# lab-cosmo/torch-pme

Hardware: AMD Instinct MI355X
Metric: atom-steps/sec (energy+forces) (higher is better)
Workload: dtype f32

## Files before the change

### torch-pme_amd/csrc/bricks.hip

```cpp
#include "bricks_device.h"

namespace mipme {
bool bricks_supported(const mipme_mesh_t* m, int dtype) {
  const size_t s = dtype == MIPME_F32 ? 4 : 8;
  const int ns[3] = {m->nx, m->ny, m->nz};
  for (int d = 0; d < 3; ++d) {
    if (ns[d] <= 2 * BRICK) return false;
    const int rem = ns[d] % BRICK;
    if (rem != 0 && rem < 4) return false;
  }
  const size_t tile = BRICK + m->order - 1;
  if (2 * size_t(m->n_channels) * tile * tile * tile * s > 60 * 1024) return false;
  if (spread_stage_rows(m->order, s) == 0) return false;
  return true;
}
int64_t bins_bytes(const mipme_mesh_t* m, int64_t N, int dtype) {
  if (!bricks_supported(m, dtype)) return 0;
  return int64_t(bins_layout(m, N, dtype).total);
}
int plane_bins_capacity(const mipme_mesh_t* m, int64_t N, int dtype) { return plane_list_capacity(m, N, dtype); }
int plane_bands(const mipme_mesh_t* m, int dtype) {
  const int rows = plane_band_rows(m, dtype);
  return rows > 0 ? m->ny / rows : 0;
}
const void* bins_epart(const mipme_mesh_t* m, int64_t N, int dtype, void* bins, int64_t* n) {
  *n = (N + 64 / kRowLanes - 1) / (64 / kRowLanes);
  return bins_view(m, N, dtype, bins).epart;
}

bool plane_spread_runs(const mipme_mesh_t* m, int64_t N, int dtype, const mipme_sr_job_t* job, const PlaneHost* ph, bool forward) {
  const int pcap = plane_list_capacity(m, N, dtype);
  const int band_rows = pcap > 0 ? plane_band_rows(m, dtype) : 0;
  const bool bands_ok = band_rows == m->ny || !job || (job->shift_format & kShiftFormatMask) == kShiftTable32;
  return ph && ph->hat && ph->slot_values && !ph->keep_mesh && forward && pcap > 0 && m->n_channels == 1 &&
         !sparse_bricks(N, make_brick_geom(m).nb) && !deterministic_mode() && N > 0 && band_rows > 0 && bands_ok;
}

static bool defer_slots_setting() {
  static const bool on = env_flag("MIPME_DEFER_SLOTS", true);
  return on;
}
bool bins_defer_slots(const mipme_mesh_t* m, int64_t N, int dtype, const mipme_sr_job_t* job, const PlaneHost* ph) {
  return defer_slots_setting() && N < kCoalescedBinAtoms && plane_spread_runs(m, N, dtype, job, ph, true);
}
SlotRider bins_slot_rider(const mipme_mesh_t* m, int64_t N, int dtype, void* bins, const void* pos, const void* q) {
  const BinsView v = bins_view(m, N, dtype, bins);
  SlotRider r;
  r.n_atoms = N;
  r.scheme = m->scheme;
  r.order = m->order;
  r.g = make_geom(m);
  r.pos = pos;
  r.q = q;
  r.dst = v.dst;
  r.rec = v.rec;
  r.wts = v.wts;
  r.qs = v.qs;
  r.codes = v.idx.codes;
  r.over_base = v.idx.over_base;
  return r;
}

template <typename T>
int bins_build(hipStream_t st, const mipme_mesh_t* m, int64_t n_atoms, const void* pos, void* bins, int* live,
               const void* q, void* atom_rec, bool plane_lists, bool defer_slots) {
  const int dtype = dtype_of<T>();
  const Geom g = make_geom(m);
  const BrickGeom bg = make_brick_geom(m);
  BinsView v = bins_view(m, n_atoms, dtype, bins);
  MIPME_REQUIRE(live, "the binning pass needs the live brick counters");
  if (plane_lists && v.idx.pcap > 0 && !deterministic_mode()) {
// ... 364 lines not shown
```

### torch-pme_amd/csrc/common.h

```cpp
#pragma once

#include <hip/hip_runtime.h>
#include <cstdarg>
#include <cstdint>
#include <cstdlib>
#include <cstdio>

#include "../../include/mipme.h"

namespace mipme {

void set_error(const char* fmt, ...);
void note_cosched_kernel(const char* name);
void note_slot_fill(int rider_atoms);
void note_cell_riders(int n);

#define MIPME_CHECK_HIP(expr)                                                                 \
  do {                                                                                        \
    hipError_t _e = (expr);                                                                   \
    if (_e != hipSuccess) {                                                                   \
      mipme::set_error("%s failed: %s (%s:%d)", #expr, hipGetErrorString(_e), __FILE__, __LINE__); \
      return MIPME_EHIP;                                                                      \
    }                                                                                         \
  } while (0)
// ... 259 lines not shown
    for (int off = 32; off > 0; off >>= 1) tot += __shfl_xor(tot, off, 64);
    if (threadIdx.x == 0) work[k] = tot;
  }
  if (threadIdx.x == 0) __hip_atomic_store(counter, 0, __ATOMIC_RELAXED, __HIP_MEMORY_SCOPE_AGENT);
}

struct SlotRider {
  int64_t n_atoms = 0;
  int per_rider = 0;
  int scheme = 0, order = 0;
  Geom g;
  const void* pos = nullptr;
  const void* q = nullptr;
  const int* dst = nullptr;
  int4* rec = nullptr;
  void* wts = nullptr;
  void* qs = nullptr;
  unsigned char* codes = nullptr;
  int64_t over_base = 0;
};

struct ConvCell {
  const void* G_deriv;
  const double* cwave;
  int64_t n_waves;
  void* wbuf;
  double* rows;
  int n_riders;
  void* rho_hat_out;
  const void* rho_hat_in;
  double* kh_rows;
  int* ticket;
  const SlotRider* slots = nullptr;
};

struct PlaneHost {
  void* hat = nullptr;
  bool keep_mesh = true;
  bool slot_values = false;
  int parts = 1;
  void* hat_more = nullptr;
  int64_t more_stride = 0;
  mutable int parts_used = 1;
  mutable bool ycols_pending = false;
};
struct RowRideHost {
  const mipme_sr_job_t* job;
  void* epart;
  int64_t first_row, n_rows;
};

__host__ __device__ __forceinline__ unsigned xcd_contiguous(unsigned wg, unsigned n_items) {
  const unsigned chunk = (n_items + 7u) >> 3;
  return (wg & 7u) * chunk + (wg >> 3);
}
__host__ __device__ __forceinline__ unsigned pad8(unsigned n) { return (n + 7u) & ~7u; }

inline const int*& skip_flag_slot() {
  static thread_local const int* p = nullptr;
  return p;
}
#define MIPME_SKIP_IF_SET(ptr)                          \
  do {                                                  \
    if ((ptr) != nullptr && *(ptr) == 1) return;        \
  } while (0)

// ... 42 lines not shown
```

### torch-pme_amd/csrc/frames.hip

```cpp
#include "frames_device.h"

namespace mipme {
template <int SCHEME, int N, typename T>
__global__ __launch_bounds__(256) void frames_bin_atoms_kernel(const FrameDev<T>* __restrict__ table) {
  const FrameDev<T>& f = table[blockIdx.y];
  if (int64_t(blockIdx.x) * 256 >= f.N) return;
  bin_atoms_body<SCHEME, N, T>(f.g, f.bg, f.bins, f.N, f.pos, f.over_brick, f.rec, f.wts, f.q, f.atom_rec, blockIdx.x, nullptr,
                               const_cast<T*>(f.spread.qs));
}

template <int N, typename T, int PFAST, bool COMPACT>
__global__ __launch_bounds__(SPREAD_THREADS, (sizeof(T) == 4 && COMPACT) ? 6 : 1) void frames_spread_rows_kernel(const FrameDev<T>* __restrict__ table) {
  const FrameDev<T>& f = table[blockIdx.y];
  const unsigned n_spread = unsigned(f.bg.nb);
  if (blockIdx.x < n_spread)
    spread_brick_body<N, T>(f.spread, blockIdx.x);
  else if (blockIdx.x - n_spread < f.n_row_blocks) {
    extern __shared__ __attribute__((aligned(16))) char smem_rows[];
    AtomRecord<T>* tab = reinterpret_cast<AtomRecord<T>*>(smem_rows);
    if constexpr (COMPACT && std::is_same<T, float>::value) {
      if (!f.rows.dist_out) {
        sr_rows_pk_body<PFAST, SPREAD_THREADS>(f.rows, blockIdx.x - n_spread, tab);
        return;
      }
// ... 107 lines not shown
                  "frame %d: the frames path needs the table shift format (1 or 2), the same for every frame", k);
  }
  return MIPME_OK;
}

template <typename T>
static int frames_table_build_t(int n_frames, const mipme_frame_t* fr, const mipme_potential_t* pot, void* host_table) {
  SRPot s;
  int rc = make_srpot(pot, s);
  if (rc) return rc;
  const int pfast = fast_rs_exponent(s);
  MIPME_REQUIRE(pot->smearing > 0 && (pfast == 1 || pfast == 6), "the frames path covers 1/r and 1/r^6 with a smearing");
  const FastRS cf = make_fast_rs(s);
  double self_c, bg_c;
  correction_terms(pot, self_c, bg_c);
  const int dtype = dtype_of<T>();
  FrameDev<T>* out = (FrameDev<T>*)host_table;
  for (int k = 0; k < n_frames; ++k) {
    const mipme_frame_t& f = fr[k];
    const mipme_mesh_t* m = &f.mesh;
    const BinsView v = bins_view(m, f.n_atoms, dtype, f.atom_bins);
    FrameDev<T> d;
    d.g = make_geom(m);
    d.bg = make_brick_geom(m);
    d.N = f.n_atoms;
    d.pos = (const T*)f.positions;
    d.q = (const T*)f.charges;
    d.bins = v.idx;
    d.bins.live = (int*)f.brick_counters;
    d.over_brick = v.over_brick;
    d.rec = v.rec;
    d.wts = (T*)v.wts;
    d.atom_rec = (AtomRecord<T>*)f.records;
    d.even = (m->order % 2) == 0;
    d.spread.g = d.g;
    d.spread.bg = d.bg;
    d.spread.C = 1;
    d.spread.bins = d.bins;
    d.spread.from_live = true;
    d.spread.rec = v.rec;
    d.spread.wts = (const T*)v.wts;
    d.spread.val = (const T*)f.charges;
    d.spread.scale = T(1);
    d.spread.mesh = (T*)f.rho_mesh;
    d.spread.stage_rows = spread_stage_rows(m->order, sizeof(T));
    d.spread.skip = nullptr;
    d.spread.det = false;
    d.spread.qs = (const T*)v.qs;
    if (frame_plane_lists(f, dtype)) {
      d.bins.plive = d.bins.live + d.bg.nb + 1;
    } else {
      d.bins.pcap = 0;
      d.bins.wmax = nullptr;
    }
    d.spread.bins = d.bins;
    d.rows = make_fused_rows_args<T>(s, cf, f.n_atoms, f.row_ptr, f.entries_shift, f.entries, nullptr, f.positions, f.records,
                                     f.cell, f.charges, nullptr, 0, f.full_list ? 0 : 1, f.full_list, 0, f.out, f.force, nullptr,
                                     f.dist_out);
    const int64_t rpb = SPREAD_THREADS / kRowLanes;
    d.n_row_blocks = unsigned((f.n_atoms + rpb - 1) / rpb);
    d.phi_mesh = (const T*)f.phi_mesh;
    d.dc = (const T*)f.dc;
    d.inv_vol = T(1.0 / m->volume);
    d.self_c = T(self_c);
    d.bg_c = T(bg_c);
    d.out = (T*)f.out;
// ... 7 lines not shown
    th.force_scale = f.full_list ? 0.5 : 1.0;
    th.seed = f.grad_seed;
    th.grad_pos = f.grad_positions;
    th.energy = f.energy;
    d.tail = make_gather_tail<T>(th, v.epart, int((f.n_atoms + 64 / kRowLanes - 1) / (64 / kRowLanes)), nullptr, nullptr);
    d.use_tail = f.use_tail != 0;
    d.rows.epart = f.use_tail ? v.epart : nullptr;
    out[k] = d;
  }
  return MIPME_OK;
}

template <typename T>
static FrameCellRec* frames_cell_recs(const void* table, int n_frames) {
  static_assert(sizeof(FrameDev<T>) % 8 == 0, "the cell records follow the frame records");
  return (FrameCellRec*)((char*)const_cast<void*>(table) + size_t(n_frames) * sizeof(FrameDev<T>));
}

template <typename T>
static int frames_forward_t(mipme_fft_plan* plan, hipStream_t st, int n_frames, const mipme_frame_t* fr, const void* table,
                            const void* G, int64_t G_stride, void* rho_all, void* hat_all, void* phi_all, void* dc_all,
                            int pfast, void* cell_work = nullptr, bool slab = false) {
  const FrameDev<T>* tb = (const FrameDev<T>*)table;
  const mipme_mesh_t* m = &fr[0].mesh;
  const BrickGeom bg = make_brick_geom(m);
  int64_t max_atoms = 0;
  for (int k = 0; k < n_frames; ++k) max_atoms = std::max<int64_t>(max_atoms, fr[k].n_atoms);
  const unsigned atom_blocks = unsigned((max_atoms + 255) / 256);
  const unsigned F = unsigned(n_frames);
  if (slab) {
    const int rcs = frames_slab_moments<T>(st, tb, n_frames, max_atoms);
    if (rcs) return rcs;
  }
  MIPME_DISPATCH_STENCIL_B(m->scheme, m->order, (frames_bin_atoms_kernel<S, N, T><<<dim3(atom_blocks, F), 256, 0, st>>>(tb)));
  MIPME_LAUNCH_CHECK();
  const int stage_rows = spread_stage_rows(m->order, sizeof(T));
  const size_t lds = spread_lds_bytes(m->order, sizeof(T), stage_rows);
  const int64_t rpb = SPREAD_THREADS / kRowLanes;
  const unsigned grid_x = unsigned(bg.nb) + unsigned((max_atoms + rpb - 1) / rpb);
  const bool compact = fr[0].shift_format == kShiftTable32;
  bool planes = fft_plan_plane_forward_ok_batched(plan);
  for (int k = 0; k < n_frames && planes; ++k) planes = frame_plane_lists(fr[k], dtype_of<T>());
  fft_plan_begin_step(plan);
  int rc0 = MIPME_OK;
  if (!planes) note_cosched_kernel("frames_spread_rows_kernel");
  if (planes) {
    PlaneArgs<T> pa;
    size_t need = 0;
    plane_lds_layout<T>(m->ny, m->nz, pa, need);
    const int64_t Mh = int64_t(m->nx) * m->ny * (m->nz / 2 + 1);
    pa.hat = (Cplx<T>*)hat_all;
    pa.parts = plane_spread_parts_setting();
    while (pa.parts > 1 && int64_t(pa.parts) * m->nx * n_frames > 128) --pa.parts;
    if (pa.parts > 1) {
      pa.hat_more = (Cplx<T>*)fft_plan_hat_parts(plan, st, kPlanePartsMax - 1);
      pa.more_stride = Mh * n_frames;
      if (!pa.hat_more) pa.parts = 1;
    }
    while ((1 << pa.logny) < m->ny) ++pa.logny;
    while ((1 << pa.loglz) < m->nz / 2) ++pa.loglz;
    const size_t rows_lds = sizeof(T) * size_t(SPREAD_WAVES) * BRICK_PTS;
    const size_t plds = need > rows_lds ? need : rows_lds;
    const unsigned pgrid_x = unsigned(m->nx) * unsigned(pa.parts) + unsigned((max_atoms + rpb - 1) / rpb);
#define MIPME_FRAMES_PLANES(PF, CO) \
  MIPME_DISPATCH_STENCIL_B(m->scheme, m->order, (frames_plane_rows_kernel<S, N, T, PF, CO><<<dim3(pgrid_x, F), SPREAD_THREADS, plds, st>>>(tb, pa, Mh)))
    note_cosched_kernel("frames_plane_rows_kernel");
    if (cell_work) {
      if ((rc0 = frames_cell_plane_rows<T>(st, m->scheme, m->order, pfast, dim3(pgrid_x, F), plds, tb, pa, Mh))) return rc0;
    } else if (pfast == 1 && compact)
      MIPME_FRAMES_PLANES(1, true);
    else if (pfast == 1)
      MIPME_FRAMES_PLANES(1, false);
    else if (compact)
      MIPME_FRAMES_PLANES(6, true);
    else
      MIPME_FRAMES_PLANES(6, false);
#undef MIPME_FRAMES_PLANES
    fft_plan_set_forward_done(plan, true, pa.parts);
  } else if (cell_work) {
    if ((rc0 = frames_cell_spread_rows<T>(st, m->scheme, m->order, pfast, dim3(grid_x, F), lds, tb))) return rc0;
  } else if (pfast == 1 && compact)
    MIPME_DISPATCH_STENCIL_B(m->scheme, m->order,
                             ((void)S, frames_spread_rows_kernel<N, T, 1, true><<<dim3(grid_x, F), SPREAD_THREADS, lds, st>>>(tb)));
  else if (pfast == 1)
    MIPME_DISPATCH_STENCIL_B(m->scheme, m->order,
                             ((void)S, frames_spread_rows_kernel<N, T, 1, false><<<dim3(grid_x, F), SPREAD_THREADS, lds, st>>>(tb)));
  else if (compact)
    MIPME_DISPATCH_STENCIL_B(m->scheme, m->order,
                             ((void)S, frames_spread_rows_kernel<N, T, 6, true><<<dim3(grid_x, F), SPREAD_THREADS, lds, st>>>(tb)));
  else
    MIPME_DISPATCH_STENCIL_B(m->scheme, m->order,
                             ((void)S, frames_spread_rows_kernel<N, T, 6, false><<<dim3(grid_x, F), SPREAD_THREADS, lds, st>>>(tb)));
  MIPME_LAUNCH_CHECK();
  bool all_tail = true;
  for (int k = 0; k < n_frames; ++k) all_tail = all_tail && fr[k].use_tail != 0;
  const int64_t n_k = xconv_blocks(plan) / n_frames;
  void* epart_k = nullptr;
  int rc;
  if (all_tail && (rc = fft_plan_tail_scratch(plan, int64_t(sizeof(double)) * n_k * n_frames, &epart_k))) return rc;
  ConvCell cc{};
  cc.wbuf = cell_work;
  rc = convolve_xfused(plan, st, rho_all, G, hat_all, phi_all, dc_all, G_stride, nullptr, nullptr, nullptr, epart_k, nullptr, 0, nullptr, nullptr,
                       cell_work ? &cc : nullptr);
  if (rc) return rc;
  const FrameCellRec* recs = frames_cell_recs<T>(table, n_frames);
  if (cell_work) {
    MIPME_REQUIRE(all_tail, "the cell gradient of a frame batch rides on the gather tail of every frame");
    const int n_riders = int(cell_work_layout(m, 1, nullptr).n_riders);
    if ((rc = frames_cell_riders<T>(st, recs, n_frames, n_riders, m->nx, m->ny, m->nz / 2 + 1, (const double*)epart_k, int(n_k)))) return rc;
  }
  if (slab) {
    MIPME_REQUIRE(all_tail, "the slab term of a frame batch rides on the gather tail of every frame");
    if ((rc = frames_slab_gather_tail<T>(st, m->scheme, m->order, dim3(unsigned(bg.nb), F), tb, (const double*)epart_k, int(n_k)))) return rc;
    return cell_work ? frames_slab_cell_finalize<T>(st, recs, n_frames) : MIPME_OK;
  }
  if (all_tail) {
    MIPME_DISPATCH_STENCIL_B(m->scheme, m->order,
                             ((void)S, frames_gather_tail_kernel<N, T><<<dim3(unsigned(bg.nb), F), GATHER_THREADS, 0, st>>>(
                                 tb, (const double*)epart_k, int(n_k))));
    MIPME_LAUNCH_CHECK();
    if (cell_work) return frames_cell_finalize<T>(st, recs, n_frames);
    return MIPME_OK;
  }
  MIPME_DISPATCH_STENCIL_B(m->scheme, m->order,
                           ((void)S, frames_gather_kernel<N, T><<<dim3(unsigned(bg.nb), F), GATHER_THREADS, 0, st>>>(tb)));
  MIPME_LAUNCH_CHECK();
  frames_energy_kernel<T><<<F, 1024, 0, st>>>(tb);
  MIPME_LAUNCH_CHECK();
  return MIPME_OK;
}

}

using namespace mipme;

template <typename T>
static int frames_table_energy_log_t(int n_frames, void* host_table, void* log, void* cursors, int capacity) {
// ... 269 lines not shown
```

### torch-pme_amd/csrc/frames_device.h

```cpp
#pragma once
#include "bricks_device.h"

namespace mipme {
template <typename T>
struct FrameDev {
  Geom g;
  BrickGeom bg;
  int64_t N;
  const T* pos;
  const T* q;
  BinIndex bins;
  int* over_brick;
  int4* rec;
  T* wts;
  AtomRecord<T>* atom_rec;
  int even;
  SpreadArgs<T> spread;
  FusedRowsArgs<T> rows;
  unsigned n_row_blocks;
  const T* phi_mesh;
  const T* dc;
  T inv_vol, self_c, bg_c;
  T* out;
  T* field;
  T* energy;
  const T* force;
  T* grad_pos;
  T force_scale;
  GatherTail<T> tail;
  bool use_tail;
};

template <typename T> int frames_cell_plane_rows(hipStream_t st, int scheme, int order, int pfast, dim3 grid, size_t lds,
                                                 const FrameDev<T>* table, const PlaneArgs<T>& pa, int64_t frame_stride);
template <typename T> int frames_cell_spread_rows(hipStream_t st, int scheme, int order, int pfast, dim3 grid, size_t lds, const FrameDev<T>* table);

template <typename T> int frames_slab_moments(hipStream_t st, const FrameDev<T>* table, int n_frames, int64_t max_atoms);
template <typename T> int frames_slab_gather_tail(hipStream_t st, int scheme, int order, dim3 grid, const FrameDev<T>* table,
                                                  const double* epart_k, int n_k);

}
```

### torch-pme_amd/csrc/host.h

```cpp
#pragma once

#include <algorithm>
#include <climits>
#include <cmath>
#include <cstring>

#include "common.h"

namespace mipme {

template <typename T>
constexpr int dtype_of() {
  return sizeof(T) == 4 ? MIPME_F32 : MIPME_F64;
}

#define DT_SWITCH(dtype, CALL_F32, CALL_F64)                    \
  do {                                                          \
    if ((dtype) == MIPME_F32) return CALL_F32;                  \
    if ((dtype) == MIPME_F64) return CALL_F64;                  \
    mipme::set_error("invalid dtype %d", int(dtype));           \
    return MIPME_EINVAL;                                        \
  } while (0)

inline unsigned stride_grid(int64_t n, int block) {
// ... 58 lines not shown
int64_t cellgrad_blocks(const mipme_mesh_t* m);
int64_t cellgrad_scratch_doubles();
template <typename T> int cellgrad_finalize_impl(hipStream_t st, const mipme_mesh_t* m, double bg, int64_t n_atoms, void* partials,
                                                 const void* pos, const void* grad_pos, const void* gout, const void* phi_atoms,
                                                 const void* rho_dc, const void* psi_dc, const void* energy_scale, void* grad_cell,
                                                 int64_t kgrid_blocks, const void* field, const void* q);
template <typename T> int cell_tail_finalize_impl(hipStream_t st, const mipme_mesh_t* m, double bg, double pair_scale, int64_t n_rows,
                                                  int64_t n_bricks, const void* rows, const void* rpart, const void* dc, const void* seed, void* out,
                                                  const GatherTailHost* slab = nullptr);

template <typename T, typename I> int rspace_forward_impl(hipStream_t st, int64_t P, int64_t N, int C, const void* pairs, const void* dist, const void* q,
                                                          const void* mask, int full, const mipme_potential_t* pot, int accumulate, void* out);
template <typename T, typename I> int rspace_backward_impl(hipStream_t st, int64_t P, int64_t N, int C, const void* pairs, const void* dist,
                                                           const void* q, const void* mask, int full, const mipme_potential_t* pot, const void* g,
                                                           const void* gscale, void* grad_d, void* grad_q);
template <typename T, typename I> int distance_forward_impl(hipStream_t st, int64_t P, const void* pairs, const void* pos, const void* cell,
                                                            const void* shifts, void* out);
template <typename T, typename I> int distance_backward_impl(hipStream_t st, int64_t P, int64_t N, const void* pairs, const void* pos, const void* cell,
                                                             const void* shifts, const void* grad_d, void* partials, void* grad_pos, void* grad_cell);
template <typename T> int pack_pair_shifts_impl(hipStream_t st, int64_t P, const void* shifts, void* packed, void* flag);
template <typename T> int distance_forward_packed_impl(hipStream_t st, int64_t P, const void* pairs, const void* packed, const void* pos,
                                                       const void* cell, void* out);
int64_t pair_partials_blocks(int64_t P);

bool bricks_supported(const mipme_mesh_t* m, int dtype);
int64_t bins_bytes(const mipme_mesh_t* m, int64_t N, int dtype);
int plane_bins_capacity(const mipme_mesh_t* m, int64_t N, int dtype);
int plane_bands(const mipme_mesh_t* m, int dtype);
const void* bins_epart(const mipme_mesh_t* m, int64_t N, int dtype, void* bins, int64_t* n);
bool sr_job_fusable(const mipme_sr_job_t* job);
template <typename T> int bins_build(hipStream_t st, const mipme_mesh_t* m, int64_t n_atoms, const void* pos, void* bins, int* live,
                                     const void* q, void* atom_rec, bool plane_lists = false, bool defer_slots = false);
bool plane_spread_runs(const mipme_mesh_t* m, int64_t N, int dtype, const mipme_sr_job_t* job, const PlaneHost* ph, bool forward);
bool bins_defer_slots(const mipme_mesh_t* m, int64_t N, int dtype, const mipme_sr_job_t* job, const PlaneHost* ph);
SlotRider bins_slot_rider(const mipme_mesh_t* m, int64_t N, int dtype, void* bins, const void* pos, const void* q);
template <typename T> int spread_bricks(hipStream_t st, const mipme_mesh_t* m, int64_t N, void* bins, const void* val, double scale, void* mesh,
                                        int* clear_count, const mipme_sr_job_t* job, bool want_epart, double* cpart, const PlaneHost* ph = nullptr,
                                        bool* used_planes = nullptr);
template <typename T> int gather_bricks(hipStream_t st, const mipme_mesh_t* m, int64_t N, void* bins, const void* mesh, const void* q,
                                        const void* qsum, double self_c, double bg_c, void* out, void* raw, int accumulate, void* field,
                                        const GatherTailHost* th, void* nan_flag, int* live);
template <typename T> int gather_grad_bricks(hipStream_t st, const mipme_mesh_t* m, int64_t N, void* bins, const void* q, const void* gout,
                                             const void* phi, const void* chi, const void* psi_dc, const void* gscale, double self_c,
                                             double bg_c, void* grad_pos, void* grad_q);

bool live_supported(const mipme_mesh_t* m, int64_t N, int dtype);
int64_t live_lists_ints(const mipme_mesh_t* m, int64_t N);
template <typename T> int live_rebin(hipStream_t st, const mipme_mesh_t* m, int64_t N, const void* rec4, void* bins, void* lists, void* host_flags);
template <typename T> int live_spread(hipStream_t st, const mipme_mesh_t* m, int64_t N, const void* rec4, void* bins, void* lists, void* mesh,
                                      const mipme_sr_job_t* job, void* host_flags, double* cpart);
template <typename T> int live_gather(hipStream_t st, const mipme_mesh_t* m, int64_t N, const void* rec4, void* bins, void* lists, const void* mesh,
                                      const void* qsum, double self_c, double bg_c, void* out, void* field, const GatherTailHost* th, void* nan_flag);

inline void correction_terms(const mipme_potential_t* pot, double& self_c, double& bg_c) {
  const int p = pot->kind == MIPME_COULOMB ? 1 : pot->exponent;
  const double two_s2 = 2.0 * pot->smearing * pot->smearing;
  self_c = pot->prefactor / std::tgamma(0.5 * p + 1.0) / std::pow(two_s2, 0.5 * p);
  if (p >= 3)
    bg_c = 0.0;
  else
    bg_c = pot->prefactor * std::pow(3.14159265358979323846, 1.5) * std::pow(two_s2, 0.5 * (3 - p)) /
           ((3 - p) * std::tgamma(0.5 * p));
}

static constexpr int kPlanePartsMax = 8;
inline int plane_spread_parts_setting() {
// ... 91 lines not shown
```

### torch-pme_amd/csrc/kfilter.hip

```cpp
#include <hipfft/hipfft.h>

#include <cmath>
#include <cstdlib>
#include <new>

#include "host.h"
#include "kgrid.h"
#include "kpot.h"
#include "fft_lds.h"
#include "cell_finalize_device.h"
#include "bricks_device.h"

namespace mipme {

struct KPoint {
  double k[3];
  int f[3];
  double G, dGdk[3], dGdh[3];
  double alpha, beta[3];
};

__device__ inline void eval_point(const KGeom& g, const KPot& kp, int ix, int iy, int iz, KPoint& o) {
  o.f[0] = fft_freq(ix, g.nx);
  o.f[1] = fft_freq(iy, g.ny);
  o.f[2] = iz;
  const double k2 = kvector_dev(g.inv, o.f, o.k);
  double v, dv;
  lr_kernel_dev(kp, k2, v, dv);
  if (g.scheme == MIPME_LAGRANGE) {
    o.G = v;
    o.alpha = 2.0 * dv;
#pragma unroll
    for (int c = 0; c < 3; ++c) {
      o.dGdk[c] = 2.0 * o.k[c] * dv;
      o.dGdh[c] = 0.0;
      o.beta[c] = 0.0;
    }
    return;
  }
  double s = 1.0, t[3], sn[3], cs[3];
#pragma unroll
  for (int c = 0; c < 3; ++c) {
    t[c] = 0.5 * o.k[c] * g.h[c];
    sincos(t[c], &sn[c], &cs[c]);
// ... 409 lines not shown

template <typename T, bool INVERSE, bool YSTAGE = true>
__global__ __launch_bounds__(1024) void yz_planes_kernel(int ny, int nz, int logny, int loglz, const T* __restrict__ real_in,
                                                       Cplx<T>* __restrict__ hat, T* __restrict__ real_out,
                                                       const int* __restrict__ skip, unsigned n_planes, CellRider rider) {
  MIPME_SKIP_IF_SET(skip);
  extern __shared__ __attribute__((aligned(16))) char smem_yz[];
  if constexpr (INVERSE && YSTAGE) {
    if (blockIdx.x >= n_planes) {
      cell_rider_body<T>(rider, blockIdx.x - n_planes, int(blockDim.x), reinterpret_cast<double*>(smem_yz));
      return;
    }
  }
  yz_plane_body<T, INVERSE, YSTAGE>(ny, nz, logny, loglz, real_in, hat, real_out, blockIdx.x, smem_yz);
}

template <int SCHEME, int N, typename T>
__global__ __launch_bounds__(1024) void yz_planes_slots_kernel(int ny, int nz, int logny, int loglz, Cplx<T>* __restrict__ hat,
                                                             T* __restrict__ real_out, const int* __restrict__ skip,
                                                             unsigned n_planes, CellRider rider, SlotRider slots) {
  MIPME_SKIP_IF_SET(skip);
  extern __shared__ __attribute__((aligned(16))) char smem_yz[];
  if (blockIdx.x >= n_planes + unsigned(rider.n_riders)) {
    slot_rider_body<SCHEME, N, T>(slots, blockIdx.x - n_planes - unsigned(rider.n_riders));
    return;
  }
  if (blockIdx.x >= n_planes) {
    cell_rider_body<T>(rider, blockIdx.x - n_planes, int(blockDim.x), reinterpret_cast<double*>(smem_yz));
    return;
  }
  yz_plane_body<T, true, true>(ny, nz, logny, loglz, nullptr, hat, real_out, blockIdx.x, smem_yz);
}

__device__ __forceinline__ unsigned xcd_tile(unsigned b, unsigned n) {
  const unsigned x = b & 7u, per = n >> 3, rem = n & 7u;
  return x * per + (x < rem ? x : rem) + (b >> 3);
}

template <typename T, bool INVERSE>
__global__ __launch_bounds__(256) void ycols_kernel(int ny, int nzh, int logny, int kzs, int nchunk, Cplx<T>* __restrict__ hat,
                                                   const int* __restrict__ skip) {
  MIPME_SKIP_IF_SET(skip);
  extern __shared__ __attribute__((aligned(16))) char smem_yc[];
  const int KZ = 1 << kzs, KP = KZ + 1;
  Cplx<T>* tile = reinterpret_cast<Cplx<T>*>(smem_yc);
  Cplx<T>* tw = tile + size_t(ny) * KP;
  const int tid = threadIdx.x, nthr = blockDim.x;
  const unsigned tile_id = xcd_tile(blockIdx.x, gridDim.x);
  const int chunk = tile_id % nchunk;
  const int64_t plane = tile_id / nchunk;
  const int kz0 = chunk << kzs, kzn = min(KZ, nzh - kz0);
  for (int j = tid; j < (ny >> 1); j += nthr) unit_root(j, ny, tw[j].re, tw[j].im);
  Cplx<T>* col = hat + plane * int64_t(ny) * nzh + kz0;
  const int n_el = ny << kzs;
  for (int idx = tid; idx < n_el; idx += nthr) {
    const int y = idx >> kzs, z = idx & (KZ - 1);
    const int yt = INVERSE ? int(__brev(unsigned(y)) >> (32 - logny)) : y;
    tile[yt * KP + z] = z < kzn ? col[int64_t(y) * nzh + z] : Cplx<T>{T(0), T(0)};
  }
  __syncthreads();
  lds_fft_radix2<T, INVERSE, INVERSE, MIPME_FFT_BFAST ? 1 : 0>(tile, logny, KZ, 1, KP, tw, ny);
  for (int idx = tid; idx < n_el; idx += nthr) {
    const int y = idx >> kzs, z = idx & (KZ - 1);
    const int ys = INVERSE ? y : int(__brev(unsigned(y)) >> (32 - logny));
    if (z < kzn) col[int64_t(ys) * nzh + z] = tile[y * KP + z];
  }
// ... 31 lines not shown
  while ((1 << loglz) < p->nz / 2) ++loglz;
  const int Lz = p->nz / 2, R = p->split_rows;
  const size_t lds = sizeof(Cplx<T>) * (size_t(R) * (Lz + 1) + size_t(Lz) / 2 + size_t(Lz + 1));
  const unsigned grid = unsigned(int64_t(p->nx) * p->ny * p->batch / R);
  const int work = R * (Lz + 1);
  const int threads = work >= 2048 ? 1024 : (work >= 512 ? 256 : 64);
  if (inverse)
    yz_planes_kernel<T, true, false><<<grid, threads, lds, st>>>(R, p->nz, 0, loglz, nullptr, (Cplx<T>*)hat, (T*)real_out, skip_flag_slot(), grid, CellRider{});
  else
    yz_planes_kernel<T, false, false><<<grid, threads, lds, st>>>(R, p->nz, 0, loglz, (const T*)real_in, (Cplx<T>*)hat, nullptr, skip_flag_slot(), grid, CellRider{});
  MIPME_LAUNCH_CHECK();
  return MIPME_OK;
}

template <typename T>
static int cell_riders_alone(hipStream_t st, const CellRider& r) {
  cell_rider_kernel<T><<<unsigned(r.n_riders), 1024, 0, st>>>(r);
  MIPME_LAUNCH_CHECK();
  return MIPME_OK;
}

static void yz_launch_shape(const mipme_fft_plan* p, size_t real_bytes, int& logny, int& loglz, size_t& lds, int& threads) {
  logny = loglz = 0;
  while ((1 << logny) < p->ny) ++logny;
  while ((1 << loglz) < p->nz / 2) ++loglz;
  const int Lz = p->nz / 2, Ltab = p->ny > Lz ? p->ny : Lz;
  lds = 2 * real_bytes * (size_t(p->ny) * (Lz + 1) + size_t(Ltab) / 2 + size_t(Lz + 1));
  const int work = p->ny * (Lz + 1);
  threads = work >= 2048 ? 1024 : (work >= 512 ? 256 : 64);
}

template <typename T>
static int yz_planes(mipme_fft_plan* p, hipStream_t st, bool inverse, const void* real_in, void* hat, void* real_out,
                     const CellRider* rider = nullptr, const SlotRider* slots = nullptr) {
  MIPME_REQUIRE(!slots || (inverse && !p->split_yz && skip_flag_slot() == nullptr),
                "slot riders need the single-launch inverse planes and a clear skip flag");
  if (p->split_yz) {
    int rc;
    if (!inverse) {
      if ((rc = zrows<T>(p, st, false, real_in, hat, nullptr))) return rc;
      return ycols<T>(p, st, false, hat);
    }
    if (rider && rider->n_riders > 0 && (rc = cell_riders_alone<T>(st, *rider))) return rc;
    if ((rc = ycols<T>(p, st, true, hat))) return rc;
    return zrows<T>(p, st, true, nullptr, hat, real_out);
  }
  int logny = 0, loglz = 0, threads = 0;
  size_t lds = 0;
  yz_launch_shape(p, sizeof(T), logny, loglz, lds, threads);
  const unsigned grid = unsigned(p->nx) * unsigned(p->batch);
  const unsigned n_riders = (inverse && rider) ? unsigned(rider->n_riders) : 0u;
  if (n_riders && lds < sizeof(double) * 16 * kCellRow) lds = sizeof(double) * 16 * kCellRow;
  if (lds > 64 * 1024) {
    static bool raised[2] = {false, false};
    if (!raised[inverse ? 1 : 0]) {
      const void* fn = inverse ? (const void*)yz_planes_kernel<T, true> : (const void*)yz_planes_kernel<T, false>;
      MIPME_CHECK_HIP(hipFuncSetAttribute(fn, hipFuncAttributeMaxDynamicSharedMemorySize, int(kYzMaxLds)));
      raised[inverse ? 1 : 0] = true;
    }
  }
  if (inverse && slots) {
    SlotRider sr = *slots;
    sr.per_rider = threads < kSlotRiderAtoms ? threads : kSlotRiderAtoms;
    const unsigned n_slot_riders = unsigned((sr.n_atoms + sr.per_rider - 1) / sr.per_rider);
    const bool raise = lds > 64 * 1024;
    int slot_rc = MIPME_OK;
    MIPME_DISPATCH_STENCIL_B(sr.scheme, sr.order, (slot_rc = [&]() -> int {
      if (raise) {
        static bool raised_slots = false;
        if (!raised_slots) {
          MIPME_CHECK_HIP(hipFuncSetAttribute((const void*)yz_planes_slots_kernel<S, N, T>, hipFuncAttributeMaxDynamicSharedMemorySize, int(kYzMaxLds)));
          raised_slots = true;
        }
      }
      yz_planes_slots_kernel<S, N, T><<<grid + n_riders + n_slot_riders, threads, lds, st>>>(
          p->ny, p->nz, logny, loglz, (Cplx<T>*)hat, (T*)real_out, skip_flag_slot(), grid, n_riders ? *rider : CellRider{}, sr);
      return MIPME_OK;
    }()));
    if (slot_rc) return slot_rc;
    note_slot_fill(sr.per_rider);
    note_cell_riders(int(n_riders));
  } else if (inverse)
    yz_planes_kernel<T, true><<<grid + n_riders, threads, lds, st>>>(p->ny, p->nz, logny, loglz, nullptr, (Cplx<T>*)hat, (T*)real_out,
                                                                     skip_flag_slot(), grid, n_riders ? *rider : CellRider{});
  else
    yz_planes_kernel<T, false><<<grid, threads, lds, st>>>(p->ny, p->nz, logny, loglz, (const T*)real_in, (Cplx<T>*)hat, nullptr,
                                                           skip_flag_slot(), grid, CellRider{});
  MIPME_LAUNCH_CHECK();
  return MIPME_OK;
}

#ifndef MIPME_X_PAD
#define MIPME_X_PAD 1
#endif
static constexpr int kXPad = MIPME_X_PAD;
struct XCellExtra {
  void* wbuf;
  void* rho_hat_out;
  const void* rho_hat_in;
  const void* hat_more = nullptr;
  int n_more = 0;
  int64_t more_stride = 0;
};
template <typename T, int CELLSUMS>
__device__ __forceinline__ void xconv_tile_body(int nx, int ny, int nzh, int log2nx, int kzs, int nchunk,
                                                Cplx<T>* __restrict__ hat, const T* __restrict__ G, int64_t G_stride,
                                                T* __restrict__ dc, const KGeom& kg, const KPot& kp,
                                                double* __restrict__ partials, double* __restrict__ epart,
                                                const double* __restrict__ sr_part, int n_sr_part, unsigned tile_id,
// ... 302 lines not shown
    rider.dG4 = cc->G_deriv;
    rider.cwave = cc->cwave;
    rider.n_waves = int(cc->n_waves);
    rider.epart_k = (const double*)epart;
    rider.n_tiles = int(grid);
    rider.rows = cc->rows;
  }
  const bool forward_done = p->forward_done, forward_ycols = p->forward_ycols;
  p->forward_done = p->forward_ycols = false;
  if (forward_done) {
    if (forward_ycols) {
      int rc = ycols<T>(p, st, false, hat);
      if (rc) return rc;
    }
  } else if (p->own_yz) {
    int rc = yz_planes<T>(p, st, false, mesh_in, hat, nullptr);
    if (rc) return rc;
  } else if (sizeof(T) == 4) {
    MIPME_CHECK_FFT(hipfftExecR2C(p->fwd2d, (hipfftReal*)mesh_in, (hipfftComplex*)hat));
  } else {
    MIPME_CHECK_FFT(hipfftExecD2Z(p->fwd2d, (hipfftDoubleReal*)mesh_in, (hipfftDoubleComplex*)hat));
  }
#define MIPME_XCONV_LAUNCH(MODE)                                                                                              \
  xconv_kernel<T, MODE><<<grid, threads, lds, st>>>(p->nx, p->ny, nzh, log2nx, kzs, nchunk, (Cplx<T>*)hat, (const T*)G,      \
                                                    G_stride, (T*)dc, kg, kp, (double*)cell_partials, (double*)epart,        \
                                                    (const double*)sr_part, int(n_sr_part), skip_flag_slot(), xc)
  if (cell_partials)
    MIPME_XCONV_LAUNCH(1);
  else
    MIPME_XCONV_LAUNCH(0);
#undef MIPME_XCONV_LAUNCH
  MIPME_LAUNCH_CHECK();
  const SlotRider* slots = (cc && cc->slots && cc->slots->n_atoms > 0) ? cc->slots : nullptr;
  MIPME_REQUIRE(!slots || (p->own_yz && p->batch == 1), "slot riders need the plan's own (y,z) plane kernels and a single mesh");
  if (p->own_yz) {
    int rc = yz_planes<T>(p, st, true, nullptr, hat, mesh_out, riders ? &rider : nullptr, slots);
    if (rc) return rc;
  } else {
    if (riders) {
      int rc = cell_riders_alone<T>(st, rider);
      if (rc) return rc;
    }
    if (sizeof(T) == 4)
      MIPME_CHECK_FFT(hipfftExecC2R(p->inv2d, (hipfftComplex*)hat, (hipfftReal*)mesh_out));
    else
      MIPME_CHECK_FFT(hipfftExecZ2D(p->inv2d, (hipfftDoubleComplex*)hat, (hipfftDoubleReal*)mesh_out));
  }
  return MIPME_OK;
}

int convolve_xfused(mipme_fft_plan* p, hipStream_t st, const void* mesh_in, const void* G, void* hat, void* mesh_out,
                    void* dc, int64_t G_stride, const mipme_mesh_t* cell_mesh, const mipme_potential_t* cell_pot,
                    void* cell_partials, void* epart, const void* sr_part, int64_t n_sr_part, const RowRideHost* rh,
                    void* err_flag, const ConvCell* cc) {
  MIPME_REQUIRE(!rh || rh->n_rows <= 0, "row riders on the convolution launches were an experiment of round 2 (tools/r06/pruned_experiments.patch)");
  if (!p->own_yz) {
    MIPME_CHECK_FFT(hipfftSetStream(p->fwd2d, st));
    MIPME_CHECK_FFT(hipfftSetStream(p->inv2d, st));
  }
  if (p->dtype == MIPME_F32)
    return convolve_xfused_t<float>(p, st, mesh_in, G, hat, mesh_out, dc, G_stride, cell_mesh, cell_pot, cell_partials, epart,
                                    sr_part, n_sr_part, cc);
  return convolve_xfused_t<double>(p, st, mesh_in, G, hat, mesh_out, dc, G_stride, cell_mesh, cell_pot, cell_partials, epart,
                                   sr_part, n_sr_part, cc);
}

bool fft_plan_plane_forward_ok(const mipme_fft_plan* p) {
  return p && p->own_yz && !p->split_yz && p->batch == 1;
}
// ... 446 lines not shown
```

Measured before the change: 593.4 million.

## Defer per-atom slot fill in frame batches to riders on inverse yz-plane FFT

For batched frames using plane lists, binning now runs a lean kernel that skips writing stencil records and weights. That per-atom slot work is moved into extra rider blocks appended to the inverse (y,z) plane FFT launch, one set of chunks per frame read from the frame table. The goal is to lighten the binning pass and overlap the slot fill with the FFT planes, which are bandwidth-bound. It adds a new kernel variant and new preconditions: no cell riders, and the batch must equal the frame count.

```diff
diff --git a/torch-pme_amd/csrc/bricks.hip b/torch-pme_amd/csrc/bricks.hip
--- a/torch-pme_amd/csrc/bricks.hip
+++ b/torch-pme_amd/csrc/bricks.hip
@@ -36,7 +36,7 @@
          !sparse_bricks(N, make_brick_geom(m).nb) && !deterministic_mode() && N > 0 && band_rows > 0 && bands_ok;
 }
 
-static bool defer_slots_setting() {
+bool defer_slots_setting() {
   static const bool on = env_flag("MIPME_DEFER_SLOTS", true);
   return on;
 }
diff --git a/torch-pme_amd/csrc/common.h b/torch-pme_amd/csrc/common.h
--- a/torch-pme_amd/csrc/common.h
+++ b/torch-pme_amd/csrc/common.h
@@ -315,6 +315,8 @@
   double* kh_rows;
   int* ticket;
   const SlotRider* slots = nullptr;
+  const void* slot_frames = nullptr;
+  int slot_n_frames = 0;
 };
 
 struct PlaneHost {
diff --git a/torch-pme_amd/csrc/frames.hip b/torch-pme_amd/csrc/frames.hip
--- a/torch-pme_amd/csrc/frames.hip
+++ b/torch-pme_amd/csrc/frames.hip
@@ -163,6 +163,7 @@
     d.rec = v.rec;
     d.wts = (T*)v.wts;
     d.atom_rec = (AtomRecord<T>*)f.records;
+    d.slot_dst = v.dst;
     d.even = (m->order % 2) == 0;
     d.spread.g = d.g;
     d.spread.bg = d.bg;
@@ -236,15 +237,22 @@
     const int rcs = frames_slab_moments<T>(st, tb, n_frames, max_atoms);
     if (rcs) return rcs;
   }
-  MIPME_DISPATCH_STENCIL_B(m->scheme, m->order, (frames_bin_atoms_kernel<S, N, T><<<dim3(atom_blocks, F), 256, 0, st>>>(tb)));
-  MIPME_LAUNCH_CHECK();
+  bool planes = fft_plan_plane_forward_ok_batched(plan);
+  for (int k = 0; k < n_frames && planes; ++k) planes = frame_plane_lists(fr[k], dtype_of<T>());
+  note_slot_fill(0);
+  const bool defer = planes && skip_flag_slot() == nullptr && !deterministic_mode() && defer_slots_setting();
+  if (defer) {
+    const int rcb = frames_bin_atoms_lean<T>(st, m->scheme, m->order, dim3(atom_blocks, F), tb);
+    if (rcb) return rcb;
+  } else {
+    MIPME_DISPATCH_STENCIL_B(m->scheme, m->order, (frames_bin_atoms_kernel<S, N, T><<<dim3(atom_blocks, F), 256, 0, st>>>(tb)));
+    MIPME_LAUNCH_CHECK();
+  }
   const int stage_rows = spread_stage_rows(m->order, sizeof(T));
   const size_t lds = spread_lds_bytes(m->order, sizeof(T), stage_rows);
   const int64_t rpb = SPREAD_THREADS / kRowLanes;
   const unsigned grid_x = unsigned(bg.nb) + unsigned((max_atoms + rpb - 1) / rpb);
   const bool compact = fr[0].shift_format == kShiftTable32;
-  bool planes = fft_plan_plane_forward_ok_batched(plan);
-  for (int k = 0; k < n_frames && planes; ++k) planes = frame_plane_lists(fr[k], dtype_of<T>());
   fft_plan_begin_step(plan);
   int rc0 = MIPME_OK;
   if (!planes) note_cosched_kernel("frames_spread_rows_kernel");
@@ -304,9 +312,19 @@
   if (all_tail && (rc = fft_plan_tail_scratch(plan, int64_t(sizeof(double)) * n_k * n_frames, &epart_k))) return rc;
   ConvCell cc{};
   cc.wbuf = cell_work;
+  SlotRider slots;
+  if (defer) {
+    slots.n_atoms = max_atoms;
+    slots.scheme = m->scheme;
+    slots.order = m->order;
+    cc.slots = &slots;
+    cc.slot_frames = tb;
+    cc.slot_n_frames = n_frames;
+  }
   rc = convolve_xfused(plan, st, rho_all, G, hat_all, phi_all, dc_all, G_stride, nullptr, nullptr, nullptr, epart_k, nullptr, 0, nullptr, nullptr,
-                       cell_work ? &cc : nullptr);
-  if (rc) return rc;
+                       (cell_work || defer) ? &cc : nullptr);
+  if (rc) return rc;
+  MIPME_REQUIRE(!defer || mipme_last_slot_fill() > 0, "the binning pass of the batch left the slot fill to riders but the inverse planes carried none");
   const FrameCellRec* recs = frames_cell_recs<T>(table, n_frames);
   if (cell_work) {
     MIPME_REQUIRE(all_tail, "the cell gradient of a frame batch rides on the gather tail of every frame");
diff --git a/torch-pme_amd/csrc/frames_device.h b/torch-pme_amd/csrc/frames_device.h
--- a/torch-pme_amd/csrc/frames_device.h
+++ b/torch-pme_amd/csrc/frames_device.h
@@ -29,7 +29,27 @@
   T force_scale;
   GatherTail<T> tail;
   bool use_tail;
+  int* slot_dst;
 };
+
+template <typename T>
+__device__ __forceinline__ SlotRider frame_slot_rider(const FrameDev<T>& f, int per_rider) {
+  SlotRider r;
+  r.n_atoms = f.N;
+  r.per_rider = per_rider;
+  r.g = f.g;
+  r.pos = f.pos;
+  r.q = f.q;
+  r.dst = f.slot_dst;
+  r.rec = f.rec;
+  r.wts = f.wts;
+  r.qs = const_cast<T*>(f.spread.qs);
+  r.codes = f.bins.codes;
+  r.over_base = f.bins.over_base;
+  return r;
+}
+
+template <typename T> int frames_bin_atoms_lean(hipStream_t st, int scheme, int order, dim3 grid, const FrameDev<T>* table);
 
 template <typename T> int frames_cell_plane_rows(hipStream_t st, int scheme, int order, int pfast, dim3 grid, size_t lds,
                                                  const FrameDev<T>* table, const PlaneArgs<T>& pa, int64_t frame_stride);
diff --git a/torch-pme_amd/csrc/frames_slots.hip b/torch-pme_amd/csrc/frames_slots.hip
--- /dev/null
+++ b/torch-pme_amd/csrc/frames_slots.hip
@@ -0,0 +1,23 @@
+#include "frames_device.h"
+
+namespace mipme {
+
+template <int SCHEME, int N, typename T>
+__global__ __launch_bounds__(256) void frames_bin_atoms_lean_kernel(const FrameDev<T>* __restrict__ table) {
+  const FrameDev<T>& f = table[blockIdx.y];
+  if (int64_t(blockIdx.x) * 256 >= f.N) return;
+  bin_atoms_body<SCHEME, N, T, false, true>(f.g, f.bg, f.bins, f.N, f.pos, f.over_brick, nullptr, nullptr, f.q, f.atom_rec, blockIdx.x,
+                                            nullptr, const_cast<T*>(f.spread.qs), f.slot_dst);
+}
+
+template <typename T>
+int frames_bin_atoms_lean(hipStream_t st, int scheme, int order, dim3 grid, const FrameDev<T>* table) {
+  MIPME_DISPATCH_STENCIL_B(scheme, order, (frames_bin_atoms_lean_kernel<S, N, T><<<grid, 256, 0, st>>>(table)));
+  MIPME_LAUNCH_CHECK();
+  return MIPME_OK;
+}
+
+template int frames_bin_atoms_lean<float>(hipStream_t, int, int, dim3, const FrameDev<float>*);
+template int frames_bin_atoms_lean<double>(hipStream_t, int, int, dim3, const FrameDev<double>*);
+
+}
diff --git a/torch-pme_amd/csrc/host.h b/torch-pme_amd/csrc/host.h
--- a/torch-pme_amd/csrc/host.h
+++ b/torch-pme_amd/csrc/host.h
@@ -114,6 +114,7 @@
 template <typename T> int bins_build(hipStream_t st, const mipme_mesh_t* m, int64_t n_atoms, const void* pos, void* bins, int* live,
                                      const void* q, void* atom_rec, bool plane_lists = false, bool defer_slots = false);
 bool plane_spread_runs(const mipme_mesh_t* m, int64_t N, int dtype, const mipme_sr_job_t* job, const PlaneHost* ph, bool forward);
+bool defer_slots_setting();
 bool bins_defer_slots(const mipme_mesh_t* m, int64_t N, int dtype, const mipme_sr_job_t* job, const PlaneHost* ph);
 SlotRider bins_slot_rider(const mipme_mesh_t* m, int64_t N, int dtype, void* bins, const void* pos, const void* q);
 template <typename T> int spread_bricks(hipStream_t st, const mipme_mesh_t* m, int64_t N, void* bins, const void* val, double scale, void* mesh,
diff --git a/torch-pme_amd/csrc/kfilter.hip b/torch-pme_amd/csrc/kfilter.hip
--- a/torch-pme_amd/csrc/kfilter.hip
+++ b/torch-pme_amd/csrc/kfilter.hip
@@ -10,6 +10,7 @@
 #include "fft_lds.h"
 #include "cell_finalize_device.h"
 #include "bricks_device.h"
+#include "frames_device.h"
 
 namespace mipme {
 
@@ -485,6 +486,23 @@
   yz_plane_body<T, true, true>(ny, nz, logny, loglz, nullptr, hat, real_out, blockIdx.x, smem_yz);
 }
 
+template <int SCHEME, int N, typename T>
+__global__ __launch_bounds__(1024) void yz_planes_frame_slots_kernel(int ny, int nz, int logny, int loglz, Cplx<T>* __restrict__ hat,
+                                                                   T* __restrict__ real_out, const int* __restrict__ skip,
+                                                                   unsigned n_planes, const FrameDev<T>* __restrict__ table,
+                                                                   int per_rider, unsigned chunks) {
+  MIPME_SKIP_IF_SET(skip);
+  extern __shared__ __attribute__((aligned(16))) char smem_yz[];
+  if (blockIdx.x >= n_planes) {
+    const unsigned r = blockIdx.x - n_planes, frame = r / chunks, chunk = r - frame * chunks;
+    const FrameDev<T>& f = table[frame];
+    if (int64_t(chunk) * per_rider >= f.N) return;
+    slot_rider_body<SCHEME, N, T>(frame_slot_rider<T>(f, per_rider), chunk);
+    return;
+  }
+  yz_plane_body<T, true, true>(ny, nz, logny, loglz, nullptr, hat, real_out, blockIdx.x, smem_yz);
+}
+
 __device__ __forceinline__ unsigned xcd_tile(unsigned b, unsigned n) {
   const unsigned x = b & 7u, per = n >> 3, rem = n & 7u;
   return x * per + (x < rem ? x : rem) + (b >> 3);
@@ -582,7 +600,8 @@
 
 template <typename T>
 static int yz_planes(mipme_fft_plan* p, hipStream_t st, bool inverse, const void* real_in, void* hat, void* real_out,
-                     const CellRider* rider = nullptr, const SlotRider* slots = nullptr) {
+                     const CellRider* rider = nullptr, const SlotRider* slots = nullptr, const void* slot_frames = nullptr,
+                     int slot_n_frames = 0) {
   MIPME_REQUIRE(!slots || (inverse && !p->split_yz && skip_flag_slot() == nullptr),
                 "slot riders need the single-launch inverse planes and a clear skip flag");
   if (p->split_yz) {
@@ -612,19 +631,28 @@
   if (inverse && slots) {
     SlotRider sr = *slots;
     sr.per_rider = threads < kSlotRiderAtoms ? threads : kSlotRiderAtoms;
-    const unsigned n_slot_riders = unsigned((sr.n_atoms + sr.per_rider - 1) / sr.per_rider);
+    const unsigned chunks = unsigned((sr.n_atoms + sr.per_rider - 1) / sr.per_rider);
+    const unsigned n_slot_riders = slot_frames ? chunks * unsigned(slot_n_frames) : chunks;
     const bool raise = lds > 64 * 1024;
     int slot_rc = MIPME_OK;
+    MIPME_REQUIRE(!slot_frames || (n_riders == 0 && slot_n_frames == p->batch),
+                  "the slot riders of a frame batch serve every mesh of the plan and share the launch with no cell riders");
     MIPME_DISPATCH_STENCIL_B(sr.scheme, sr.order, (slot_rc = [&]() -> int {
       if (raise) {
-        static bool raised_slots = false;
-        if (!raised_slots) {
-          MIPME_CHECK_HIP(hipFuncSetAttribute((const void*)yz_planes_slots_kernel<S, N, T>, hipFuncAttributeMaxDynamicSharedMemorySize, int(kYzMaxLds)));
-          raised_slots = true;
+        static bool raised_slots[2] = {false, false};
+        const void* fn = slot_frames ? (const void*)yz_planes_frame_slots_kernel<S, N, T> : (const void*)yz_planes_slots_kernel<S, N, T>;
+        if (!raised_slots[slot_frames ? 1 : 0]) {
+          MIPME_CHECK_HIP(hipFuncSetAttribute(fn, hipFuncAttributeMaxDynamicSharedMemorySize, int(kYzMaxLds)));
+          raised_slots[slot_frames ? 1 : 0] = true;
         }
       }
-      yz_planes_slots_kernel<S, N, T><<<grid + n_riders + n_slot_riders, threads, lds, st>>>(
-          p->ny, p->nz, logny, loglz, (Cplx<T>*)hat, (T*)real_out, skip_flag_slot(), grid, n_riders ? *rider : CellRider{}, sr);
+      if (slot_frames)
+        yz_planes_frame_slots_kernel<S, N, T><<<grid + n_slot_riders, threads, lds, st>>>(
+            p->ny, p->nz, logny, loglz, (Cplx<T>*)hat, (T*)real_out, skip_flag_slot(), grid, (const FrameDev<T>*)slot_frames,
+            sr.per_rider, chunks);
+      else
+        yz_planes_slots_kernel<S, N, T><<<grid + n_riders + n_slot_riders, threads, lds, st>>>(
+            p->ny, p->nz, logny, loglz, (Cplx<T>*)hat, (T*)real_out, skip_flag_slot(), grid, n_riders ? *rider : CellRider{}, sr);
       return MIPME_OK;
     }()));
     if (slot_rc) return slot_rc;
@@ -993,9 +1021,11 @@
 #undef MIPME_XCONV_LAUNCH
   MIPME_LAUNCH_CHECK();
   const SlotRider* slots = (cc && cc->slots && cc->slots->n_atoms > 0) ? cc->slots : nullptr;
-  MIPME_REQUIRE(!slots || (p->own_yz && p->batch == 1), "slot riders need the plan's own (y,z) plane kernels and a single mesh");
+  MIPME_REQUIRE(!slots || (p->own_yz && (p->batch == 1 || cc->slot_frames)),
+                "slot riders need the plan's own (y,z) plane kernels and a single mesh or a frame batch's table");
   if (p->own_yz) {
-    int rc = yz_planes<T>(p, st, true, nullptr, hat, mesh_out, riders ? &rider : nullptr, slots);
+    int rc = yz_planes<T>(p, st, true, nullptr, hat, mesh_out, riders ? &rider : nullptr, slots, slots ? cc->slot_frames : nullptr,
+                          slots ? cc->slot_n_frames : 0);
     if (rc) return rc;
   } else {
     if (riders) {
```

Result: no change. 590.6 million, median of 2 (-0.5%).
